# caburu/gym-supplychain

Measured on AMD Instinct MI355X. Metric: env-steps/sec at 65536 envs/GPU, beergame-v0; 1/2/4/8 MI355X, higher is better.
Workload: dtype int32; 1 GPU; beergame-v0 step() x 65536 envs/GPU (BASELINE configs[1]; configs[4] at N=8); n_envs_per_gpu=65536, levels=4, weeks=35, auto_reset=True, ledgers=True, orders_history=True, episode_return_allgather=False, parallelism=env-shard x1

## Files before the change

gym-supplychain_amd/csrc/scg_beergame.hip:

```cpp

#include <cstdarg>
#include <cstdio>
#include <ctime>
#include <vector>

#include "scg_beergame_kernels.h"
#include "scg_server_host.h"

namespace scg {

__global__ __launch_bounds__(kBlock) void poisson_demand_kernel(const BgArgs a, int32_t weeks,
                                                                int32_t* __restrict__ out) {
  const int64_t n = static_cast<int64_t>(blockIdx.x) * kBlock + threadIdx.x;
  if (n >= a.n) return;
  for (int32_t w = 1; w <= weeks; ++w) out[(int64_t)(w - 1) * a.n + n] = week_demand(a, n, w, a.episode);
}

__global__ __launch_bounds__(kBlock) void uniform_ints_kernel(uint32_t k0, uint32_t k1, int64_t env_offset,
                                                              int64_t n_envs, int32_t rows, int32_t width,
                                                              uint32_t tag, int32_t lo, uint32_t range,
                                                              int32_t* __restrict__ out) {
  const int64_t n = static_cast<int64_t>(blockIdx.x) * kBlock + threadIdx.x;
  if (n >= n_envs) return;
  const uint32_t env = static_cast<uint32_t>(env_offset + n);
// ... 19 lines not shown
  if (q < SCG_BG_MAX_LEVELS) dst->init_inv[q] = v.init_inv[q];
  if (q != 63) return;
  dst->env_base = v.env_base;
  dst->pthr_len = v.pthr_len;
  dst->h = v.h;
  dst->b = v.b;
  dst->guard = v.guard;
  dst->demand_lo = v.demand_lo;
  dst->demand_hi = v.demand_hi;
  dst->ship_value = v.ship_value;
  dst->orders_value = v.orders_value;
  dst->init_slots = v.init_slots;
  dst->err_host = v.err_host;
  dst->demand_table = v.demand_table;
  dst->pthr = v.pthr;
}

template <class F>
int with_level(int L, F&& f) {
#define X(l) bg_launchers<l>,
  static const BgLaunchers* (*const kLevels[])() = {SCG_LEVEL_CASES(X)};
#undef X
  if (L < 1 || L > SCG_BG_MAX_LEVELS) return fail(SCG_ERR_INVALID, "levels=%d outside 1..%d", L, SCG_BG_MAX_LEVELS);
  return f(*kLevels[L - 1]());
}

int slab_layout(int L, int64_t N, int32_t R, int32_t T, bool history, int64_t* off) {
  const int64_t NL = N * L;
  if (NL % 4 != 0) return fail(SCG_ERR_INVALID, "slab layout needs n_envs * levels %% 4 == 0 (got %lld)", (long long)NL);
  if (R < 1 || R > static_cast<int32_t>(kSlabRingMax)) return fail(SCG_ERR_INVALID, "slab layout needs 1 <= ring_slots <= 127");
// ... 116 lines not shown
  std::memcpy(w, &v, sizeof(w));
  uint64_t h = 0x9E3779B97F4A7C15ull ^ reinterpret_cast<uintptr_t>(block);
  for (uint64_t x : w) {
    h = (h ^ x) * 0xFF51AFD7ED558CCDull;
    h ^= h >> 29;
  }
  return h | 1u;
}

int sync_slab_consts(const scg_bg_config* cfg, scg_bg_state* st, hipStream_t s) {
  const BgSlabConst v = slab_consts(cfg, st);
  const uint64_t tag = slab_consts_tag(v, st->step_consts);
  if (tag == st->step_consts_tag) return SCG_OK;
  if (reinterpret_cast<uintptr_t>(st->step_consts) % alignof(BgSlabConst) != 0)
    return fail(SCG_ERR_INVALID, "step_consts must be %d-byte aligned", static_cast<int>(alignof(BgSlabConst)));
  hipLaunchKernelGGL(bg_slab_consts_kernel, dim3(1), dim3(64), 0, s, static_cast<BgSlabConst*>(st->step_consts), v);
  if (int rc = check_launch("bg_slab_consts_kernel")) return rc;
  st->step_consts_tag = tag;
  return SCG_OK;
}

}

using namespace scg;

extern "C" {

int scg_bg_struct_sizes(size_t* config_size, size_t* state_size) {
  if (config_size) *config_size = sizeof(scg_bg_config);
  if (state_size) *state_size = sizeof(scg_bg_state);
  return SCG_OK;
// ... 117 lines not shown
  } else {
    st->week = wk.week;
  }
}

static int check_step(const scg_bg_config* cfg, const scg_bg_state* st) {
  if (st->week < 0) return fail(SCG_ERR_NOT_RESET, "step() before reset()");
  if (st->week >= cfg->max_weeks)
    return fail(SCG_ERR_PAST_HORIZON, "step() after the terminal week %d (customer_demand has %d weeks)",
                cfg->max_weeks, cfg->max_weeks);
  return SCG_OK;
}

int scg_bg_step(const scg_bg_config* cfg, scg_bg_state* st, const int32_t* action, int32_t* obs,
                int32_t* reward, int32_t* terminal_obs, uint32_t flags, int32_t* done, void* stream) {
  return scg_bg_step_timed(cfg, st, action, obs, reward, terminal_obs, flags, done, nullptr, nullptr, stream);
}

int scg_bg_step_timed(const scg_bg_config* cfg, scg_bg_state* st, const int32_t* action, int32_t* obs,
                      int32_t* reward, int32_t* terminal_obs, uint32_t flags, int32_t* done, void* start_event,
                      void* stop_event, void* stream) {
  if (int rc = check_state(cfg, st)) return rc;
  if (!action || !obs || !reward) return fail(SCG_ERR_INVALID, "action/obs/reward buffers are required");
  if (int rc = check_step(cfg, st)) return rc;
  const int32_t w = st->week + 1;
  const WeekInfo wk = week_info(cfg, w, flags);
  const dim3 grid = grid_for(st->n_envs);
  const hipStream_t s = static_cast<hipStream_t>(stream);
  const hipEvent_t ev0 = static_cast<hipEvent_t>(start_event), ev1 = static_cast<hipEvent_t>(stop_event);
  if (slab_ready(cfg, st, obs, reward, terminal_obs)) {
    if (int rc = sync_slab_consts(cfg, st, s)) return rc;
    const uint32_t wpack = pack_week_slab(wk, cfg->ring_slots, st->inventory_costs != nullptr,
                                          st->episode_return != nullptr, st->orders_history != nullptr);
    const SlabLaunch sl{st->slab, action, obs, static_cast<const BgSlabConst*>(st->step_consts), st->seed,
                        static_cast<uint32_t>(st->n_envs), wpack, static_cast<uint32_t>(w), st->episode,
                        wk.demand_fixed};
    if (int rc = with_level(cfg->levels, [&](const BgLaunchers& k) { return k.slab(cfg->demand_mode, grid, s, sl, ev0, ev1); }))
      return rc;
  } else {
    BgArgs a = make_args(cfg, st);
    a.act = action;
    a.obs = obs;
    a.rew = reward;
    a.term_obs = terminal_obs;
    if (int rc = with_level(cfg->levels, [&](const BgLaunchers& k) {
          return cfg->variant == 2 ? k.step2(grid, s, a, wk) : k.step(grid, s, a, wk, ev0, ev1);
        }))
      return rc;
  }
  advance_week(st, wk);
  if (done) *done = (wk.flags & WEEK_TERMINAL) ? 1 : 0;
  return SCG_OK;
}

// ... 368 lines not shown
```

gym-supplychain_amd/csrc/scg_beergame_kernels.h:

```cpp
#pragma once

#include <hip/hip_ext.h>
#include <hip/hip_runtime.h>

#include <algorithm>
#include <cmath>
#include <cstdint>
#include <cstdlib>
#include <cstring>
#include <type_traits>

#include "scg_bg_local.h"
#include "scg_bg_mlp.h"
#include "scg_bg_plan.h"
#include "scg_bg_policy.h"
#include "scg_common.h"
#include "scg_mailbox.h"
#include "scg_const.h"
#include "scg_philox.h"
#include "scgpu.h"

namespace scg {

constexpr int kBlock = 256;
// ... 510 lines not shown
  __builtin_amdgcn_fence(__ATOMIC_RELEASE, "");
  if (lane == 0) __hip_atomic_store(&box->exit_seq, ex, __ATOMIC_RELEASE, __HIP_MEMORY_SCOPE_SYSTEM);
}

struct alignas(64) BgSlabConst {
  uint32_t env_base;
  int32_t pthr_len;
  int32_t h, b, guard;
  int32_t demand_lo, demand_hi;
  int32_t ship_value, orders_value, init_slots;
  int32_t* err_host;
  const int32_t* demand_table;
  const uint32_t* pthr;
  int32_t init_inv[SCG_BG_MAX_LEVELS];
  uint32_t thr[kFastThr];
};
static_assert(sizeof(BgSlabConst) <= SCG_BG_STEP_CONSTS_BYTES && offsetof(BgSlabConst, err_host) == 40 &&
                  offsetof(BgSlabConst, init_inv) == 64 && offsetof(BgSlabConst, thr) == 128,
              "BgSlabConst layout");

constexpr int kSlabHeader = 4;

template <int L, int DM>
__global__ __launch_bounds__(kBlock) void bg_step_slab_kernel(int32_t* __restrict__ slab, const int32_t* __restrict__ act_p,
                                                              int32_t* __restrict__ out,
                                                              const BgSlabConst* __restrict__ consts, uint64_t key,
                                                              uint32_t n32, uint32_t wpack, uint32_t week,
                                                              uint32_t episode, int32_t demand_fixed) {
  const int64_t n = static_cast<int64_t>(blockIdx.x) * kBlock + threadIdx.x;
  if (n >= static_cast<int64_t>(n32)) return;
  const ConstTab<BgSlabConst> c = const_tab(consts);
  const uint32_t key0 = static_cast<uint32_t>(key), key1 = static_cast<uint32_t>(key >> 32);
  const WeekPlan p = unpack_week_slab(wpack);
  const int32_t read_slot = p.read_slot, write_slot = p.write_slot, mode = p.mode, R = p.R;
  const bool terminal = p.terminal, autoreset = p.autoreset;
  const bool ledgers = p.ledgers, returns = p.returns, history = p.history;
  const int64_t NL = static_cast<int64_t>(n32) * L;
  const int64_t row = n * L;
  int32_t* const rows = slab + kSlabHeader;
  int32_t* const inv_p = rows, *const bk_p = rows + NL, *const op_p = rows + 2 * NL;
  int32_t* const iacc_p = rows + 3 * NL, *const bacc_p = rows + 4 * NL, *const term_p = rows + 5 * NL;
  int32_t* const ring_p = rows + 6 * NL;
  int64_t* const ret_p = reinterpret_cast<int64_t*>(rows + (6 + R) * NL);
  int64_t* const fret_p = ret_p + n32;
  int32_t* const hist_p = reinterpret_cast<int32_t*>(fret_p + n32);

  int32_t inv[L], bk[L], op[L], act[L], due[L], cur[L], iacc[L], bacc[L];
  zero_row<L>(due);
  zero_row<L>(cur);
  zero_row<L>(iacc);
  zero_row<L>(bacc);
  load_row<L>(inv_p + row, inv);
  load_row<L>(bk_p + row, bk);
  load_row<L>(op_p + row, op);
  load_row<L>(act_p + row, act);
  if (read_slot >= 0) load_row<L>(ring_p + read_slot * NL + row, due);
  if (mode == MODE_ADD) load_row<L>(ring_p + write_slot * NL + row, cur);
  if (ledgers && !autoreset) {
    load_row<L>(iacc_p + row, iacc);
    load_row<L>(bacc_p + row, bacc);
  }
// ... 11 lines not shown
  } else if constexpr (DM == SCG_DEMAND_UNIFORM) {
    const int32_t lo = c->demand_lo, hi = c->demand_hi;
    uint32_t env_base = c->env_base;
    asm volatile("" : "+s"(env_base) : "s"(lo), "s"(hi), "s"(h), "s"(b), "s"(guard), "s"(err_host));
    const uint32_t w = scg::philox_word(key0, key1, env_base + static_cast<uint32_t>(n), episode, week - 1,
                                        SCG_STREAM_BG2_DEMAND);
    demand = lo + static_cast<int32_t>((static_cast<uint64_t>(w) * static_cast<uint32_t>(hi - lo)) >> 32);
  } else {
    static_assert(kFastThr == 40, "the thresholds are read as 16 + 16 + 8 dwords");
    const u32x16 t0 = *reinterpret_cast<ConstTab<u32x16>>(c->thr);
    const u32x16 t1 = *reinterpret_cast<ConstTab<u32x16>>(c->thr + 16);
    const u32x8 t2 = *reinterpret_cast<ConstTab<u32x8>>(c->thr + 32);
    const int32_t len = c->pthr_len;
    const ConstTab<uint32_t> pthr = const_tab(c->pthr);
    uint32_t env_base = c->env_base;
    asm volatile("" : "+s"(env_base) : "s"(t0), "s"(t1), "s"(t2), "s"(len), "s"(pthr), "s"(h), "s"(b), "s"(guard),
                 "s"(err_host));
    uint32_t fast[kFastThr];
#pragma unroll
    for (int q = 0; q < 16; ++q) fast[q] = t0[q], fast[16 + q] = t1[q];
#pragma unroll
    for (int q = 0; q < 8; ++q) fast[32 + q] = t2[q];
    const uint32_t u = scg::philox_word(key0, key1, env_base + static_cast<uint32_t>(n), episode, week - 1,
                                        SCG_STREAM_DEMAND);
    demand = poisson_count_padded(fast, pthr, len, u);
  }
  export_error(n, terminal, slab, err_host);

  int32_t ship[L], obs[L];
  bool ovf = false;
  const int32_t reward = week_update<L>(h, b, guard, demand, mode == MODE_DIRECT, due, inv, bk, op, act, ship,
                                        obs, cur, iacc, bacc, ovf);
  if (mode == MODE_STORE) {
    store_row_p<L>(ring_p + write_slot * NL + row, ship);
  } else if (mode == MODE_ADD) {
    store_row_p<L>(ring_p + write_slot * NL + row, cur);
  }
  out[NL + n] = reward;
  if (history) store_row_p<L>(hist_p + static_cast<int64_t>(week) * NL + row, op);
  const int64_t ret = ret0 + reward;
// ... 646 lines not shown
```

gym-supplychain_amd/csrc/scg_bg_plan.h:

```cpp
#pragma once

#include <cstdint>

#include "scgpu.h"

#if defined(__HIPCC__)
#define SCG_PLAN_HD __host__ __device__ __attribute__((always_inline)) inline
#else
#define SCG_PLAN_HD inline
#endif

namespace scg {

enum : int32_t { MODE_DIRECT = 0, MODE_STORE = 1, MODE_ADD = 2, MODE_DROP = 3 };
constexpr int32_t PLAN_ARRIVE = 4;
inline int32_t plan_mode(int32_t p) { return p & 3; }
inline bool plan_arrive(int32_t p) { return (p & PLAN_ARRIVE) != 0; }
constexpr int kPlanDelayShift = 8;
static_assert(static_cast<int64_t>(SCG_BG_MAX_DELAY) << kPlanDelayShift <= INT32_MAX, "plan delay field too narrow");
inline int32_t plan_word(int32_t mode, bool arrive, int32_t delay) {
  return mode | (arrive ? PLAN_ARRIVE : 0) | (delay << kPlanDelayShift);
}
inline int32_t plan_delay(int32_t p) { return p >> kPlanDelayShift; }

// ... 2 lines not shown
  int32_t week;
  int32_t read_slot;
  int32_t write_slot;
  int32_t mode;
  int32_t demand_fixed;
  int32_t flags;
};

struct WeekPlan {
  int32_t read_slot;
  int32_t write_slot;
  int32_t mode;
  uint32_t terminal, autoreset;
  int32_t R;
  uint32_t ledgers, returns, history;
};

constexpr uint32_t kWeekSlotBits = 14, kWeekSlotMask = (1u << kWeekSlotBits) - 1;
constexpr uint32_t kWeekModeShift = 2 * kWeekSlotBits, kWeekFlagsShift = kWeekModeShift + 2;
static_assert(SCG_BG_MAX_WEEKS + SCG_BG_MAX_DELAY + 2 < (1 << kWeekSlotBits), "ring slot field too narrow");
static_assert(kWeekFlagsShift + 2 == 32 && MODE_DROP <= 3 && (WEEK_TERMINAL | WEEK_AUTORESET) <= 3, "week word fields");
SCG_PLAN_HD uint32_t pack_week(const WeekInfo& wk) {
  return static_cast<uint32_t>(wk.read_slot + 1) | (static_cast<uint32_t>(wk.write_slot) << kWeekSlotBits) |
         (static_cast<uint32_t>(wk.mode) << kWeekModeShift) | (static_cast<uint32_t>(wk.flags) << kWeekFlagsShift);
}
SCG_PLAN_HD WeekPlan unpack_week(uint32_t w) {
  WeekPlan p{};
  p.read_slot = static_cast<int32_t>(w & kWeekSlotMask) - 1;
  p.write_slot = static_cast<int32_t>((w >> kWeekSlotBits) & kWeekSlotMask);
  p.mode = static_cast<int32_t>((w >> kWeekModeShift) & 3u);
  p.terminal = w & (static_cast<uint32_t>(WEEK_TERMINAL) << kWeekFlagsShift);
  p.autoreset = w & (static_cast<uint32_t>(WEEK_AUTORESET) << kWeekFlagsShift);
  return p;
}

constexpr uint32_t kSlabSlotBits = 8, kSlabSlotMask = (1u << kSlabSlotBits) - 1;
constexpr uint32_t kSlabModeShift = 2 * kSlabSlotBits, kSlabRingShift = 24, kSlabRingMax = 127;
constexpr uint32_t SW_TERMINAL = 1u << 18, SW_AUTORESET = 1u << 19, SW_LEDGERS = 1u << 20, SW_RETURNS = 1u << 21,
                   SW_HISTORY = 1u << 22;
static_assert(kSlabRingMax <= kSlabSlotMask && (3u << kSlabModeShift) < SW_TERMINAL &&
                  SW_HISTORY < (1u << kSlabRingShift) && (kSlabRingMax << kSlabRingShift) >> kSlabRingShift == kSlabRingMax,
              "slab week word fields");
SCG_PLAN_HD uint32_t pack_week_slab(const WeekInfo& wk, int32_t R, bool ledgers, bool returns, bool history) {
  return static_cast<uint32_t>(wk.read_slot + 1) | (static_cast<uint32_t>(wk.write_slot) << kSlabSlotBits) |
         (static_cast<uint32_t>(wk.mode) << kSlabModeShift) | ((wk.flags & WEEK_TERMINAL) ? SW_TERMINAL : 0u) |
         ((wk.flags & WEEK_AUTORESET) ? SW_AUTORESET : 0u) | (ledgers ? SW_LEDGERS : 0u) |
         (returns ? SW_RETURNS : 0u) | (history ? SW_HISTORY : 0u) | (static_cast<uint32_t>(R) << kSlabRingShift);
}
SCG_PLAN_HD WeekPlan unpack_week_slab(uint32_t w) {
  WeekPlan p{};
  p.read_slot = static_cast<int32_t>(w & kSlabSlotMask) - 1;
  p.write_slot = static_cast<int32_t>((w >> kSlabSlotBits) & kSlabSlotMask);
  p.mode = static_cast<int32_t>((w >> kSlabModeShift) & 3u);
  p.R = static_cast<int32_t>((w >> kSlabRingShift) & kSlabRingMax);
  p.terminal = w & SW_TERMINAL;
  p.autoreset = w & SW_AUTORESET;
  p.ledgers = w & SW_LEDGERS;
  p.returns = w & SW_RETURNS;
  p.history = w & SW_HISTORY;
  return p;
}

}
```

gym-supplychain_amd/csrc/scg_pybind.c:

```c
#define PY_SSIZE_T_CLEAN
#include <Python.h>
#include <stdint.h>
#include <time.h>

#include "scgpu.h"

static int as_ptr(PyObject* o, void** out) {
  if (o == Py_None) {
    *out = NULL;
    return 0;
  }
  unsigned long long v = PyLong_AsUnsignedLongLong(o);
  if (v == (unsigned long long)-1 && PyErr_Occurred()) return -1;
  *out = (void*)(uintptr_t)v;
  return 0;
}

static PyObject* bg_step(PyObject* self, PyObject* const* args, Py_ssize_t nargs) {
  (void)self;
  void* p[8];
  if (nargs != 8) {
    PyErr_SetString(PyExc_TypeError, "bg_step expects 8 arguments");
    return NULL;
  }
  for (int i = 0; i < 8; ++i)
    if (as_ptr(args[i], &p[i])) return NULL;
  int32_t done = 0;
  const int rc = scg_bg_step((const scg_bg_config*)p[0], (scg_bg_state*)p[1], (const int32_t*)p[2], (int32_t*)p[3],
                             (int32_t*)p[4], (int32_t*)p[5], (uint32_t)(uintptr_t)p[6], &done, p[7]);
  return PyLong_FromLong((long)((rc << 1) | (done ? 1 : 0)));
}

typedef struct bg_step_args {
  uint64_t cfg, state, obs, reward, terminal_obs;
  uint32_t flags;
} bg_step_args;

static PyObject* bg_step_h(PyObject* self, PyObject* const* args, Py_ssize_t nargs) {
  (void)self;
  void* p[3];
  if (nargs != 3) {
    PyErr_SetString(PyExc_TypeError, "bg_step_h expects 3 arguments");
    return NULL;
  }
  for (int i = 0; i < 3; ++i)
    if (as_ptr(args[i], &p[i])) return NULL;
  const bg_step_args* h = (const bg_step_args*)p[0];
  if (!h) {
    PyErr_SetString(PyExc_ValueError, "bg_step_h: null handle");
    return NULL;
  }
  int32_t done = 0;
  const int rc = scg_bg_step((const scg_bg_config*)(uintptr_t)h->cfg, (scg_bg_state*)(uintptr_t)h->state,
                             (const int32_t*)p[1], (int32_t*)(uintptr_t)h->obs, (int32_t*)(uintptr_t)h->reward,
                             (int32_t*)(uintptr_t)h->terminal_obs, h->flags, &done, p[2]);
  return PyLong_FromLong((long)((rc << 1) | (done ? 1 : 0)));
}

static PyObject* bg_step_timed(PyObject* self, PyObject* const* args, Py_ssize_t nargs) {
  (void)self;
  void* p[10];
  if (nargs != 10) {
    PyErr_SetString(PyExc_TypeError, "bg_step_timed expects 10 arguments");
    return NULL;
  }
  for (int i = 0; i < 10; ++i)
    if (as_ptr(args[i], &p[i])) return NULL;
  int32_t done = 0;
  const int rc = scg_bg_step_timed((const scg_bg_config*)p[0], (scg_bg_state*)p[1], (const int32_t*)p[2],
                                   (int32_t*)p[3], (int32_t*)p[4], (int32_t*)p[5], (uint32_t)(uintptr_t)p[6], &done,
                                   p[7], p[8], p[9]);
  return PyLong_FromLong((long)((rc << 1) | (done ? 1 : 0)));
}

static PyObject* bg_server_step(PyObject* self, PyObject* const* args, Py_ssize_t nargs) {
  (void)self;
  void* p[3];
  if (nargs != 3) {
    PyErr_SetString(PyExc_TypeError, "bg_server_step expects 3 arguments");
    return NULL;
  }
  for (int i = 0; i < 3; ++i)
    if (as_ptr(args[i], &p[i])) return NULL;
  scg_bg_state* st = (scg_bg_state*)p[1];
  scg_bg_server_slot* slot = (scg_bg_server_slot*)p[2];
  int32_t done = 0;
// ... 85 lines not shown
      __builtin_ia32_pause();
    }
  }
  Py_END_ALLOW_THREADS
  if (timed_out) {
    PyErr_SetString(PyExc_TimeoutError, "node_barrier: not every rank arrived");
    return NULL;
  }
  return PyLong_FromLong(sense);
}

static PyMethodDef methods[] = {
    {"bg_step", (PyCFunction)(void (*)(void))bg_step, METH_FASTCALL, "scg_bg_step"},
    {"bg_step_h", (PyCFunction)(void (*)(void))bg_step_h, METH_FASTCALL, "scg_bg_step with the fixed arguments behind a handle"},
    {"bg_server_step", (PyCFunction)(void (*)(void))bg_server_step, METH_FASTCALL, "scg_bg_server_step"},
    {"bg_step_timed", (PyCFunction)(void (*)(void))bg_step_timed, METH_FASTCALL, "scg_bg_step_timed"},
    {"sc_step", (PyCFunction)(void (*)(void))sc_step, METH_FASTCALL, "scg_sc_step"},
    {"sc_server_step", (PyCFunction)(void (*)(void))sc_server_step, METH_FASTCALL, "scg_sc_server_post + _wait"},
    {"node_barrier", (PyCFunction)(void (*)(void))node_barrier, METH_FASTCALL, "host barrier of one node's ranks"},
    {NULL, NULL, 0, NULL},
};

static struct PyModuleDef module = {PyModuleDef_HEAD_INIT, "_scgpu_fast", NULL, -1, methods,
                                    NULL, NULL, NULL, NULL};

PyMODINIT_FUNC PyInit__scgpu_fast(void) { return PyModule_Create(&module); }
```

gym-supplychain_amd/gym_supplychain_amd/_native.py:

```python
import ctypes
import os

import torch

LIB_NAME = "libscgpu.so"
LIB_PATH = os.path.join(os.path.dirname(os.path.abspath(__file__)), LIB_NAME)
ABI_VERSION = 9

SCG_OK = 0
SCG_ERR_INVALID = 1
SCG_ERR_PAST_HORIZON = 2
SCG_ERR_NOT_RESET = 3
SCG_ERR_HIP = 4
SCG_PENDING = 5

SCG_DEMAND_FIXED = 0
SCG_DEMAND_TABLE = 1
SCG_DEMAND_POISSON = 2
SCG_DEMAND_UNIFORM = 3

SCG_BG_AUTORESET = 1
SCG_SC_SERIAL = 2
SCG_SC_LAST_OBS = 8
SCG_STREAM_DEMAND = 0
# ... 61 lines not shown
        ("inventory_costs", ctypes.c_void_p),
        ("backlog_costs", ctypes.c_void_p),
        ("orders_history", ctypes.c_void_p),
        ("episode_return", ctypes.c_void_p),
        ("final_return", ctypes.c_void_p),
        ("penalty_costs", ctypes.c_void_p),
        ("error_flags", ctypes.c_void_p),
        ("error_host", ctypes.c_void_p),
        ("slab", ctypes.c_void_p),
        ("step_consts", ctypes.c_void_p),
        ("step_consts_tag", ctypes.c_uint64),
    ]


BG_STEP_CONSTS_BYTES = 512


BG_SERVER_SLOTS = 15
BG_SERVER_ARGS_BYTES = 512


class BgPolicy(ctypes.Structure):
    _fields_ = [("kind", ctypes.c_int32), ("shift", ctypes.c_int32), ("act_lo", ctypes.c_int32),
                ("act_hi", ctypes.c_int32), ("params", ctypes.c_void_p)]


class BgLocalPolicy(ctypes.Structure):
    _fields_ = [("kind", ctypes.c_int32), ("shift", ctypes.c_int32), ("act_lo", ctypes.c_int32),
                ("act_hi", ctypes.c_int32), ("params", ctypes.c_void_p)]

# ... 142 lines not shown
SIGNATURES = {
    "scg_abi_version": (ctypes.c_int, []),
    "scg_last_error": (ctypes.c_char_p, []),
    "scg_bg_struct_sizes": (ctypes.c_int, [ctypes.POINTER(ctypes.c_size_t), ctypes.POINTER(ctypes.c_size_t)]),
    "scg_poisson_table": (ctypes.c_int, [ctypes.c_double, _u32p, ctypes.c_int32]),
    "scg_bg_prepare": (ctypes.c_int, [ctypes.POINTER(BgConfig)]),
    "scg_bg_slab_layout": (ctypes.c_int, [ctypes.POINTER(BgConfig), ctypes.c_int64, ctypes.c_int32, _i64p]),
    "scg_bg_reset": (ctypes.c_int, [ctypes.POINTER(BgConfig), ctypes.POINTER(BgState), ctypes.c_void_p,
                                    ctypes.c_void_p]),
    "scg_bg_step": (ctypes.c_int, [ctypes.POINTER(BgConfig), ctypes.POINTER(BgState), ctypes.c_void_p,
                                   ctypes.c_void_p, ctypes.c_void_p, ctypes.c_void_p, ctypes.c_uint32,
                                   _i32p, ctypes.c_void_p]),
    "scg_bg_step_timed": (ctypes.c_int, [ctypes.POINTER(BgConfig), ctypes.POINTER(BgState), ctypes.c_void_p,
                                         ctypes.c_void_p, ctypes.c_void_p, ctypes.c_void_p, ctypes.c_uint32,
                                         _i32p, ctypes.c_void_p, ctypes.c_void_p, ctypes.c_void_p]),
    "scg_bg_server_attach": (ctypes.c_int, [ctypes.POINTER(BgServer), ctypes.POINTER(BgServerSlot)]),
    "scg_bg_server_detach": (ctypes.c_int, [ctypes.POINTER(BgServerSlot)]),
    "scg_bg_server_post": (ctypes.c_int, [ctypes.POINTER(BgConfig), ctypes.POINTER(BgState),
                                          ctypes.POINTER(BgServerSlot)]),
    "scg_bg_server_wait": (ctypes.c_int, [ctypes.POINTER(BgState), ctypes.POINTER(BgServerSlot), ctypes.c_int64,
                                          _i32p]),
    "scg_bg_server_step": (ctypes.c_int, [ctypes.POINTER(BgConfig), ctypes.POINTER(BgState),
                                          ctypes.POINTER(BgServerSlot), _i32p]),
    "scg_bg_server_stop": (ctypes.c_int, [ctypes.POINTER(BgServer)]),
    "scg_bg_server_line_check": (ctypes.c_uint32, [ctypes.POINTER(BgServerLine)]),
    "scg_bg_rollout": (ctypes.c_int, [ctypes.POINTER(BgConfig), ctypes.POINTER(BgState), ctypes.c_int32,
                                      ctypes.c_void_p, ctypes.c_void_p, ctypes.c_void_p, ctypes.c_uint32,
                                      ctypes.c_void_p]),
    "scg_bg_rollout_policy": (ctypes.c_int, [ctypes.POINTER(BgConfig), ctypes.POINTER(BgState), ctypes.c_int32,
                                             ctypes.POINTER(BgPolicy), ctypes.c_void_p, ctypes.c_void_p,
# ... 109 lines not shown
    buf = (ctypes.c_uint32 * POISSON_MAX)()
    n = lib.scg_poisson_table(float(lam), buf, POISSON_MAX)
    if n < 0:
        check(-n)
    return list(buf[:n])


try:
    _raw_stream = torch._C._cuda_getCurrentRawStream
except AttributeError:
    _raw_stream = None


class BgStepArgs(ctypes.Structure):
    _fields_ = [("cfg", ctypes.c_uint64), ("state", ctypes.c_uint64), ("obs", ctypes.c_uint64),
                ("reward", ctypes.c_uint64), ("terminal_obs", ctypes.c_uint64), ("flags", ctypes.c_uint32)]


def raw_stream(device_index):
    if _raw_stream is not None:
        return _raw_stream(device_index)
    return torch.cuda.current_stream(device_index).cuda_stream


def raw_stream_fn():
    return _raw_stream if _raw_stream is not None else raw_stream


_hip = None


# ... 111 lines not shown
```

gym-supplychain_amd/gym_supplychain_amd/envs/beergame_env.py:

```python
import ctypes
import numbers
import os
import threading
import weakref

import numpy as np
import torch

from .. import _native as nat
from .. import checkpoint as ckpt
from .. import spaces
from . import resident
from .step_server import _ResidentServer
from .supplychain_env import SupplyChainVecEnv, pack_mlp_words
from ..distributed import entropy_seed

STD_LEVELS = 4
STD_DEMAND = [4] * 4 + [8] * 31
STD_INVENTORY = 12
STD_SHIP_DELAY = 2
STD_SHIP_VALUE = 4
STD_ORDERS_VALUE = 4
STD_INV_COST = 1
STD_BACKLOG_COST = 2
# ... 196 lines not shown
            self._final_ret = i64(nat.SLAB_FINAL_RETURN) if track_returns else None
            self._term_obs = rows(nat.SLAB_TERMINAL_OBS)
        else:
            self._err = torch.zeros(1, **i32)
            self._inv = torch.zeros((n_envs, L), **i32)
            self._bk = torch.zeros((n_envs, L), **i32)
            self._op = torch.zeros((n_envs, L), **i32)
            self._ring = torch.zeros((R, n_envs, L), **i32)
            self._inv_costs = torch.zeros((n_envs, L), **i32) if track_costs else None
            self._bk_costs = torch.zeros((n_envs, L), **i32) if track_costs else None
            self._hist = torch.zeros((T + 1, n_envs, L), **i32) if track_history else None
            self._ret = torch.zeros(n_envs, dtype=torch.int64, device=dev) if track_returns else None
            self._final_ret = torch.zeros(n_envs, dtype=torch.int64, device=dev) if track_returns else None
            self._term_obs = torch.zeros((n_envs, L), **i32)
        self._pen_costs = torch.zeros((n_envs, L), **i32) if (track_costs and v2) else None
        self._out = torch.zeros(n_envs * L + n_envs, **i32)
        self._obs = self._out[: n_envs * L].view(n_envs, L)
        self._rew = self._out[n_envs * L:]
        self._done_false = torch.zeros(n_envs, dtype=torch.bool, device=dev)
        self._done_true = torch.ones(n_envs, dtype=torch.bool, device=dev)
        self._err_word = nat.MappedWord()

        s = nat.BgState()
        s.n_envs, s.env_offset, s.seed = n_envs, int(env_offset), int(seed) & 0xFFFFFFFFFFFFFFFF
        s.episode, s.week = 0, -1
        s.inventory, s.backlog, s.orders_placed = self._inv.data_ptr(), self._bk.data_ptr(), self._op.data_ptr()
        s.shipments = self._ring.data_ptr()
        s.inventory_costs = self._inv_costs.data_ptr() if track_costs else None
        s.backlog_costs = self._bk_costs.data_ptr() if track_costs else None
        s.orders_history = self._hist.data_ptr() if track_history else None
        s.episode_return = self._ret.data_ptr() if track_returns else None
# ... 1 lines not shown
        s.penalty_costs = self._pen_costs.data_ptr() if self._pen_costs is not None else None
        s.error_flags = self._err.data_ptr()
        s.error_host = self._err_word.dev
        s.slab = self._slab.data_ptr() if self._slab is not None else None
        s.step_consts = self._step_consts.data_ptr() if self._step_consts is not None else None
        s.step_consts_tag = 0
        self._st = s
        self._cfg_ref = ctypes.byref(self._cfg)
        self._st_ref = ctypes.byref(self._st)
        self._done_flag = ctypes.c_int32(0)
        self._done_ref = ctypes.byref(self._done_flag)
        self._flags = nat.SCG_BG_AUTORESET if self.auto_reset else 0
        self._act_shape = (n_envs, L)
        self._obs_ptr, self._rew_ptr = self._obs.data_ptr(), self._rew.data_ptr()
        self._term_ptr = self._term_obs.data_ptr()
        self._cfg_addr, self._st_addr = ctypes.addressof(self._cfg), ctypes.addressof(self._st)
        self._fast_step, self._fast_step_timed = nat.fast.bg_step, nat.fast.bg_step_timed
        self._step_args = nat.BgStepArgs(self._cfg_addr, self._st_addr, self._obs_ptr, self._rew_ptr, self._term_ptr,
                                         self._flags)
        self._step_handle = ctypes.addressof(self._step_args)
        self._fast_step_h = nat.fast.bg_step_h
        self._raw_stream = nat.raw_stream_fn()
        self._ready = {}
        self._act_numel = n_envs * L
        self.single_observation_space = spaces.Box(_I32[0], _I32[1], (L,), np.int32)
        self.single_action_space = spaces.Box(-ACTION_BOUND, ACTION_BOUND - 1, (L,), np.int32)
        self.observation_space = spaces.Box(_I32[0], _I32[1], (n_envs, L), np.int32)
        self.action_space = spaces.Box(-ACTION_BOUND, ACTION_BOUND - 1, (n_envs, L), np.int32)

    def _stream(self):
        return nat.raw_stream(self._dev_index)

    def reset(self):
        nat.check(nat.lib.scg_bg_reset(self._cfg_ref, self._st_ref, self._obs.data_ptr(), self._stream()))
# ... 27 lines not shown
                and actions.numel() == self._act_numel:
            ptr = ok[1]
        else:
            if self._is_ready(actions):
                if len(self._ready) >= 64:
                    self._ready.clear()
                self._ready[id(actions)] = (weakref.ref(actions), actions.data_ptr())
            else:
                actions = self._actions(actions)
            ptr = actions.data_ptr()
        if _events is None:
            r = self._fast_step_h(self._step_handle, ptr, self._raw_stream(self._dev_index))
        else:
            r = self._fast_step_timed(self._cfg_addr, self._st_addr, ptr, self._obs_ptr,
                                      self._rew_ptr, self._term_ptr, self._flags, _events[0], _events[1],
                                      nat.raw_stream(self._dev_index))
        if r > 1:
            nat.check(r >> 1)
        if r & 1:
            self._poll_errors()
            info = {"terminal_observation": self._term_obs}
            if self._final_ret is not None:
                info["episode_return"] = self._final_ret
            return self._obs, self._rew, self._done_true, info
        return self._obs, self._rew, self._done_false, {}

    def _poll_errors(self):
        if self._err_word.value:
            raise OverflowError("a BeerGame value left int32 range (the reference's int64 state would differ); "
                                "results since then are invalid")

# ... 352 lines not shown
        self.initial_orders_value = cfg.initial_orders_value
        self.current_state = None
        ra = (4 * L + 15) // 16 * 16
        self._io = io = nat.MappedBuffer(16 + ra + 4 * (L + 1))
        self._err_np = io.view(np.int32, 0, 1)
        self._act_np = io.view(np.int32, 16, L)
        self._out_np = io.view(np.int32, 16 + ra, L + 1)
        self._act_dev = io.dev + 16
        vec = self._vec
        vec._st.error_flags = io.dev
        vec._err = torch.from_numpy(self._err_np)
        obs_dev, rew_dev = io.dev + 16 + ra, io.dev + 16 + ra + 4 * L
        self._server = None
        if os.environ.get("SCG_BG_SERVER", "1") != "0":
            self._server = _StepServer.attach(self._vec, self._act_dev, io.host + 16, obs_dev, rew_dev)
        self._step_args = nat.BgStepArgs(vec._cfg_addr, vec._st_addr, obs_dev, rew_dev, vec._term_ptr, 0)
        self._handle = ctypes.addressof(self._step_args)
        self._fast_step_h = nat.fast.bg_step_h
        self._sync = nat.stream_synchronize_fn()
        self._last_act = None
        self.week = None

    def reset(self):
        obs = self._vec.reset()
        self.week = 0
        self._last_act = None
        self.current_state = obs[0].cpu().numpy().astype(np.int64)
        return self.current_state

    def step(self, action):
        if self.week is None:
# ... 271 lines not shown
```

include/scgpu.h:

```cpp
#ifndef SCGPU_H
#define SCGPU_H

#include <stddef.h>
#include <stdint.h>

#ifdef __cplusplus
extern "C" {
#endif

#define SCG_ABI_VERSION 9

#if defined(__GNUC__)
#define SCG_API __attribute__((visibility("default")))
#else
#define SCG_API
#endif

#define SCG_BG_MAX_LEVELS 16
#define SCG_BG_MAX_WEEKS 4096
#define SCG_BG_MAX_DELAY 4096
#define SCG_POISSON_MAX 256
#define SCG_BG_ROLLOUT_MAX 128

typedef enum scg_status {
// ... 98 lines not shown

SCG_API int scg_bg_prepare(scg_bg_config* cfg);

SCG_API int scg_bg_slab_layout(const scg_bg_config* cfg, int64_t n_envs, int32_t with_history,
                               int64_t offsets[SCG_SLAB_FIELDS]);

SCG_API int scg_bg_reset(const scg_bg_config* cfg, scg_bg_state* st, int32_t* obs, void* stream);

SCG_API int scg_bg_step(const scg_bg_config* cfg, scg_bg_state* st, const int32_t* action,
                int32_t* obs, int32_t* reward, int32_t* terminal_obs, uint32_t flags,
                int32_t* done, void* stream);

SCG_API int scg_bg_step_timed(const scg_bg_config* cfg, scg_bg_state* st, const int32_t* action,
                              int32_t* obs, int32_t* reward, int32_t* terminal_obs, uint32_t flags,
                              int32_t* done, void* start_event, void* stop_event, void* stream);

#define SCG_BG_SERVER_SLOTS 15
#define SCG_BG_SERVER_ARGS_BYTES 512
#define SCG_PENDING 5

typedef struct scg_bg_server_line {
  uint32_t req_seq;
  int32_t cmd;
  uint32_t wpack;
  int32_t week;
  int32_t demand_fixed;
  int32_t n_inline;
  uint32_t gen;
  uint32_t check;
  int32_t action[8];
// ... 326 lines not shown
```

Baseline: 15.34 billion env-steps/s.

## Precompute next week's Poisson demand in extra blocks of the step kernel

The slab step kernel is launched with twice the grid for Poisson demand. The extra blocks draw the next week's demand into a double-banked 'ahead' buffer, tagged with key, env base, episode, week and an upload stamp. On the next step the main blocks check the tag and reuse the pre-drawn value, falling back to the inline Philox+Poisson draw on a mismatch. This takes the RNG and inverse-CDF work off the step's critical path, at the cost of more blocks per launch, an extra global read per env, and added tag-validation complexity.

```diff
diff --git a/gym-supplychain_amd/csrc/scg_beergame.hip b/gym-supplychain_amd/csrc/scg_beergame.hip
--- a/gym-supplychain_amd/csrc/scg_beergame.hip
+++ b/gym-supplychain_amd/csrc/scg_beergame.hip
@@ -1,4 +1,5 @@
 
+#include <atomic>
 #include <cstdarg>
 #include <cstdio>
 #include <ctime>
@@ -57,6 +58,7 @@
   dst->err_host = v.err_host;
   dst->demand_table = v.demand_table;
   dst->pthr = v.pthr;
+  dst->stamp = v.stamp;
 }
 
 template <class F>
@@ -203,7 +205,10 @@
   if (tag == st->step_consts_tag) return SCG_OK;
   if (reinterpret_cast<uintptr_t>(st->step_consts) % alignof(BgSlabConst) != 0)
     return fail(SCG_ERR_INVALID, "step_consts must be %d-byte aligned", static_cast<int>(alignof(BgSlabConst)));
-  hipLaunchKernelGGL(bg_slab_consts_kernel, dim3(1), dim3(64), 0, s, static_cast<BgSlabConst*>(st->step_consts), v);
+  static std::atomic<uint32_t> uploads{0};
+  BgSlabConst up = v;
+  do up.stamp = uploads.fetch_add(1, std::memory_order_relaxed) + 1; while (up.stamp == 0);
+  hipLaunchKernelGGL(bg_slab_consts_kernel, dim3(1), dim3(64), 0, s, static_cast<BgSlabConst*>(st->step_consts), up);
   if (int rc = check_launch("bg_slab_consts_kernel")) return rc;
   st->step_consts_tag = tag;
   return SCG_OK;
@@ -351,30 +356,42 @@
 
 int scg_bg_step(const scg_bg_config* cfg, scg_bg_state* st, const int32_t* action, int32_t* obs,
                 int32_t* reward, int32_t* terminal_obs, uint32_t flags, int32_t* done, void* stream) {
-  return scg_bg_step_timed(cfg, st, action, obs, reward, terminal_obs, flags, done, nullptr, nullptr, stream);
+  return scg_bg_step_ex(cfg, st, action, obs, reward, terminal_obs, flags, done, nullptr, nullptr, nullptr, stream);
 }
 
 int scg_bg_step_timed(const scg_bg_config* cfg, scg_bg_state* st, const int32_t* action, int32_t* obs,
                       int32_t* reward, int32_t* terminal_obs, uint32_t flags, int32_t* done, void* start_event,
                       void* stop_event, void* stream) {
+  return scg_bg_step_ex(cfg, st, action, obs, reward, terminal_obs, flags, done, start_event, stop_event, nullptr,
+                        stream);
+}
+
+int scg_bg_step_ex(const scg_bg_config* cfg, scg_bg_state* st, const int32_t* action, int32_t* obs,
+                   int32_t* reward, int32_t* terminal_obs, uint32_t flags, int32_t* done, void* start_event,
+                   void* stop_event, int32_t* ahead, void* stream) {
   if (int rc = check_state(cfg, st)) return rc;
   if (!action || !obs || !reward) return fail(SCG_ERR_INVALID, "action/obs/reward buffers are required");
   if (int rc = check_step(cfg, st)) return rc;
   const int32_t w = st->week + 1;
   const WeekInfo wk = week_info(cfg, w, flags);
-  const dim3 grid = grid_for(st->n_envs);
   const hipStream_t s = static_cast<hipStream_t>(stream);
   const hipEvent_t ev0 = static_cast<hipEvent_t>(start_event), ev1 = static_cast<hipEvent_t>(stop_event);
   if (slab_ready(cfg, st, obs, reward, terminal_obs)) {
     if (int rc = sync_slab_consts(cfg, st, s)) return rc;
+    const bool rows = ahead && ahead == reward + st->n_envs && cfg->demand_mode == SCG_DEMAND_POISSON &&
+                      st->n_envs <= kAheadMaxEnvs;
     const uint32_t wpack = pack_week_slab(wk, cfg->ring_slots, st->inventory_costs != nullptr,
-                                          st->episode_return != nullptr, st->orders_history != nullptr);
+                                          st->episode_return != nullptr, st->orders_history != nullptr, rows,
+                                          demand_bank(st->episode, cfg->max_weeks, w));
+    const bool draw = rows && !((wk.flags & WEEK_TERMINAL) && !(wk.flags & WEEK_AUTORESET));
+    const dim3 grid(draw ? 2 * grid_for(st->n_envs).x : grid_for(st->n_envs).x);
     const SlabLaunch sl{st->slab, action, obs, static_cast<const BgSlabConst*>(st->step_consts), st->seed,
                         static_cast<uint32_t>(st->n_envs), wpack, static_cast<uint32_t>(w), st->episode,
                         wk.demand_fixed};
     if (int rc = with_level(cfg->levels, [&](const BgLaunchers& k) { return k.slab(cfg->demand_mode, grid, s, sl, ev0, ev1); }))
       return rc;
   } else {
+    const dim3 grid = grid_for(st->n_envs);
     BgArgs a = make_args(cfg, st);
     a.act = action;
     a.obs = obs;
diff --git a/gym-supplychain_amd/csrc/scg_beergame_kernels.h b/gym-supplychain_amd/csrc/scg_beergame_kernels.h
--- a/gym-supplychain_amd/csrc/scg_beergame_kernels.h
+++ b/gym-supplychain_amd/csrc/scg_beergame_kernels.h
@@ -548,12 +548,52 @@
   const uint32_t* pthr;
   int32_t init_inv[SCG_BG_MAX_LEVELS];
   uint32_t thr[kFastThr];
+  uint32_t stamp;
 };
 static_assert(sizeof(BgSlabConst) <= SCG_BG_STEP_CONSTS_BYTES && offsetof(BgSlabConst, err_host) == 40 &&
-                  offsetof(BgSlabConst, init_inv) == 64 && offsetof(BgSlabConst, thr) == 128,
+                  offsetof(BgSlabConst, init_inv) == 64 && offsetof(BgSlabConst, thr) == 128 &&
+                  offsetof(BgSlabConst, stamp) == 288 && sizeof(BgSlabConst) == 320,
               "BgSlabConst layout");
 
 constexpr int kSlabHeader = 4;
+
+constexpr int kAheadHeader = SCG_BG_AHEAD_HEADER, kAheadTagWords = 7, kAheadPathWord = SCG_BG_AHEAD_PATH_WORD;
+enum : int { TAG_KEY0 = 0, TAG_KEY1, TAG_ENV_BASE, TAG_N, TAG_EPISODE, TAG_WEEK, TAG_STAMP };
+constexpr int64_t kAheadMaxEnvs = 65536;
+static_assert(8 + kAheadTagWords <= kAheadPathWord && kAheadPathWord < kAheadHeader, "two tags and the path word");
+
+__device__ __forceinline__ void draw_ahead(ConstTab<BgSlabConst> c, int32_t* __restrict__ ahead, uint32_t key0,
+                                           uint32_t key1, uint32_t n32, const WeekPlan& p, uint32_t week,
+                                           uint32_t episode, int64_t n) {
+  if (n >= static_cast<int64_t>(n32)) return;
+  static_assert(kFastThr == 40, "the thresholds are read as 16 + 16 + 8 dwords");
+  const u32x16 t0 = *reinterpret_cast<ConstTab<u32x16>>(c->thr);
+  const u32x16 t1 = *reinterpret_cast<ConstTab<u32x16>>(c->thr + 16);
+  const u32x8 t2 = *reinterpret_cast<ConstTab<u32x8>>(c->thr + 32);
+  const int32_t len = c->pthr_len;
+  const ConstTab<uint32_t> pthr = const_tab(c->pthr);
+  const uint32_t env_base = c->env_base, stamp = c->stamp;
+  const uint32_t next_week = p.terminal ? 1u : week + 1, next_episode = p.terminal ? episode + 1 : episode;
+  uint32_t fast[kFastThr];
+#pragma unroll
+  for (int q = 0; q < 16; ++q) fast[q] = t0[q], fast[16 + q] = t1[q];
+#pragma unroll
+  for (int q = 0; q < 8; ++q) fast[32 + q] = t2[q];
+  const uint32_t u = scg::philox_word(key0, key1, env_base + static_cast<uint32_t>(n), next_episode, next_week - 1,
+                                      SCG_STREAM_DEMAND);
+  const uint32_t bank = p.bank ^ 1u;
+  ahead[kAheadHeader + static_cast<int64_t>(bank) * n32 + n] = poisson_count_padded(fast, pthr, len, u);
+  if (n == 0) {
+    uint32_t* const tag = reinterpret_cast<uint32_t*>(ahead) + 8 * bank;
+    tag[TAG_KEY0] = key0;
+    tag[TAG_KEY1] = key1;
+    tag[TAG_ENV_BASE] = env_base;
+    tag[TAG_N] = n32;
+    tag[TAG_EPISODE] = next_episode;
+    tag[TAG_WEEK] = next_week;
+    tag[TAG_STAMP] = stamp;
+  }
+}
 
 template <int L, int DM>
 __global__ __launch_bounds__(kBlock) void bg_step_slab_kernel(int32_t* __restrict__ slab, const int32_t* __restrict__ act_p,
@@ -561,11 +601,19 @@
                                                               const BgSlabConst* __restrict__ consts, uint64_t key,
                                                               uint32_t n32, uint32_t wpack, uint32_t week,
                                                               uint32_t episode, int32_t demand_fixed) {
-  const int64_t n = static_cast<int64_t>(blockIdx.x) * kBlock + threadIdx.x;
-  if (n >= static_cast<int64_t>(n32)) return;
   const ConstTab<BgSlabConst> c = const_tab(consts);
   const uint32_t key0 = static_cast<uint32_t>(key), key1 = static_cast<uint32_t>(key >> 32);
   const WeekPlan p = unpack_week_slab(wpack);
+  int32_t* const ahead = out + (static_cast<int64_t>(n32) * L + n32);
+  if constexpr (DM == SCG_DEMAND_POISSON) {
+    const uint32_t G = (n32 + kBlock - 1) / kBlock;
+    if (blockIdx.x >= G) {
+      draw_ahead(c, ahead, key0, key1, n32, p, week, episode, static_cast<int64_t>(blockIdx.x - G) * kBlock + threadIdx.x);
+      return;
+    }
+  }
+  const int64_t n = static_cast<int64_t>(blockIdx.x) * kBlock + threadIdx.x;
+  if (n >= static_cast<int64_t>(n32)) return;
   const int32_t read_slot = p.read_slot, write_slot = p.write_slot, mode = p.mode, R = p.R;
   const bool terminal = p.terminal, autoreset = p.autoreset;
   const bool ledgers = p.ledgers, returns = p.returns, history = p.history;
@@ -579,6 +627,9 @@
   int64_t* const fret_p = ret_p + n32;
   int32_t* const hist_p = reinterpret_cast<int32_t*>(fret_p + n32);
 
+  int32_t drawn = 0;
+  if constexpr (DM == SCG_DEMAND_POISSON)
+    if (p.ahead) drawn = ahead[kAheadHeader + static_cast<int64_t>(p.bank) * n32 + n];
   int32_t inv[L], bk[L], op[L], act[L], due[L], cur[L], iacc[L], bacc[L];
   zero_row<L>(due);
   zero_row<L>(cur);
@@ -620,16 +671,27 @@
     const int32_t len = c->pthr_len;
     const ConstTab<uint32_t> pthr = const_tab(c->pthr);
     uint32_t env_base = c->env_base;
+    const uint32_t stamp = c->stamp;
+    const u32x8 tag = *reinterpret_cast<ConstTab<u32x8>>(
+        p.ahead ? const_tab(reinterpret_cast<const uint32_t*>(ahead) + 8 * p.bank) : static_cast<ConstTab<uint32_t>>(c->thr));
     asm volatile("" : "+s"(env_base) : "s"(t0), "s"(t1), "s"(t2), "s"(len), "s"(pthr), "s"(h), "s"(b), "s"(guard),
-                 "s"(err_host));
-    uint32_t fast[kFastThr];
-#pragma unroll
-    for (int q = 0; q < 16; ++q) fast[q] = t0[q], fast[16 + q] = t1[q];
-#pragma unroll
-    for (int q = 0; q < 8; ++q) fast[32 + q] = t2[q];
-    const uint32_t u = scg::philox_word(key0, key1, env_base + static_cast<uint32_t>(n), episode, week - 1,
-                                        SCG_STREAM_DEMAND);
-    demand = poisson_count_padded(fast, pthr, len, u);
+                 "s"(err_host), "s"(stamp), "s"(tag));
+    const uint32_t miss = (tag[TAG_KEY0] ^ key0) | (tag[TAG_KEY1] ^ key1) | (tag[TAG_ENV_BASE] ^ env_base) |
+                          (tag[TAG_N] ^ n32) | (tag[TAG_EPISODE] ^ episode) | (tag[TAG_WEEK] ^ week) |
+                          (tag[TAG_STAMP] ^ stamp) | (p.ahead ^ SW_AHEAD);
+    if (miss == 0) {
+      demand = drawn;
+    } else {
+      uint32_t fast[kFastThr];
+#pragma unroll
+      for (int q = 0; q < 16; ++q) fast[q] = t0[q], fast[16 + q] = t1[q];
+#pragma unroll
+      for (int q = 0; q < 8; ++q) fast[32 + q] = t2[q];
+      const uint32_t u = scg::philox_word(key0, key1, env_base + static_cast<uint32_t>(n), episode, week - 1,
+                                          SCG_STREAM_DEMAND);
+      demand = poisson_count_padded(fast, pthr, len, u);
+    }
+    if (p.ahead && n == 0) ahead[kAheadPathWord] = miss == 0 ? 1 : 0;
   }
   export_error(n, terminal, slab, err_host);
 
diff --git a/gym-supplychain_amd/csrc/scg_bg_plan.h b/gym-supplychain_amd/csrc/scg_bg_plan.h
--- a/gym-supplychain_amd/csrc/scg_bg_plan.h
+++ b/gym-supplychain_amd/csrc/scg_bg_plan.h
@@ -40,6 +40,7 @@
   uint32_t terminal, autoreset;
   int32_t R;
   uint32_t ledgers, returns, history;
+  uint32_t ahead, bank;
 };
 
 constexpr uint32_t kWeekSlotBits = 14, kWeekSlotMask = (1u << kWeekSlotBits) - 1;
@@ -63,15 +64,23 @@
 constexpr uint32_t kSlabSlotBits = 8, kSlabSlotMask = (1u << kSlabSlotBits) - 1;
 constexpr uint32_t kSlabModeShift = 2 * kSlabSlotBits, kSlabRingShift = 24, kSlabRingMax = 127;
 constexpr uint32_t SW_TERMINAL = 1u << 18, SW_AUTORESET = 1u << 19, SW_LEDGERS = 1u << 20, SW_RETURNS = 1u << 21,
-                   SW_HISTORY = 1u << 22;
+                   SW_HISTORY = 1u << 22, SW_AHEAD = 1u << 23, SW_BANK = 1u << 31;
 static_assert(kSlabRingMax <= kSlabSlotMask && (3u << kSlabModeShift) < SW_TERMINAL &&
                   SW_HISTORY < (1u << kSlabRingShift) && (kSlabRingMax << kSlabRingShift) >> kSlabRingShift == kSlabRingMax,
               "slab week word fields");
-SCG_PLAN_HD uint32_t pack_week_slab(const WeekInfo& wk, int32_t R, bool ledgers, bool returns, bool history) {
+static_assert(SW_HISTORY < SW_AHEAD && SW_AHEAD < (1u << kSlabRingShift) &&
+                  ((kSlabRingMax << kSlabRingShift) & SW_BANK) == 0 && SW_BANK == 1u << 31,
+              "slab week word: the demand-row bits lie between the SW_* bits and R, and above R");
+SCG_PLAN_HD uint32_t demand_bank(uint32_t episode, int32_t max_weeks, int32_t week) {
+  return (episode * static_cast<uint32_t>(max_weeks) + static_cast<uint32_t>(week)) & 1u;
+}
+SCG_PLAN_HD uint32_t pack_week_slab(const WeekInfo& wk, int32_t R, bool ledgers, bool returns, bool history,
+                                    bool ahead = false, uint32_t bank = 0) {
   return static_cast<uint32_t>(wk.read_slot + 1) | (static_cast<uint32_t>(wk.write_slot) << kSlabSlotBits) |
          (static_cast<uint32_t>(wk.mode) << kSlabModeShift) | ((wk.flags & WEEK_TERMINAL) ? SW_TERMINAL : 0u) |
          ((wk.flags & WEEK_AUTORESET) ? SW_AUTORESET : 0u) | (ledgers ? SW_LEDGERS : 0u) |
-         (returns ? SW_RETURNS : 0u) | (history ? SW_HISTORY : 0u) | (static_cast<uint32_t>(R) << kSlabRingShift);
+         (returns ? SW_RETURNS : 0u) | (history ? SW_HISTORY : 0u) | (ahead ? SW_AHEAD : 0u) |
+         ((bank & 1u) ? SW_BANK : 0u) | (static_cast<uint32_t>(R) << kSlabRingShift);
 }
 SCG_PLAN_HD WeekPlan unpack_week_slab(uint32_t w) {
   WeekPlan p{};
@@ -84,6 +93,8 @@
   p.ledgers = w & SW_LEDGERS;
   p.returns = w & SW_RETURNS;
   p.history = w & SW_HISTORY;
+  p.ahead = w & SW_AHEAD;
+  p.bank = w >> 31;
   return p;
 }
 
diff --git a/gym-supplychain_amd/csrc/scg_pybind.c b/gym-supplychain_amd/csrc/scg_pybind.c
--- a/gym-supplychain_amd/csrc/scg_pybind.c
+++ b/gym-supplychain_amd/csrc/scg_pybind.c
@@ -34,6 +34,7 @@
 typedef struct bg_step_args {
   uint64_t cfg, state, obs, reward, terminal_obs;
   uint32_t flags;
+  uint64_t ahead;
 } bg_step_args;
 
 static PyObject* bg_step_h(PyObject* self, PyObject* const* args, Py_ssize_t nargs) {
@@ -51,25 +52,26 @@
     return NULL;
   }
   int32_t done = 0;
-  const int rc = scg_bg_step((const scg_bg_config*)(uintptr_t)h->cfg, (scg_bg_state*)(uintptr_t)h->state,
-                             (const int32_t*)p[1], (int32_t*)(uintptr_t)h->obs, (int32_t*)(uintptr_t)h->reward,
-                             (int32_t*)(uintptr_t)h->terminal_obs, h->flags, &done, p[2]);
+  const int rc = scg_bg_step_ex((const scg_bg_config*)(uintptr_t)h->cfg, (scg_bg_state*)(uintptr_t)h->state,
+                                (const int32_t*)p[1], (int32_t*)(uintptr_t)h->obs, (int32_t*)(uintptr_t)h->reward,
+                                (int32_t*)(uintptr_t)h->terminal_obs, h->flags, &done, NULL, NULL,
+                                (int32_t*)(uintptr_t)h->ahead, p[2]);
   return PyLong_FromLong((long)((rc << 1) | (done ? 1 : 0)));
 }
 
 static PyObject* bg_step_timed(PyObject* self, PyObject* const* args, Py_ssize_t nargs) {
   (void)self;
-  void* p[10];
-  if (nargs != 10) {
-    PyErr_SetString(PyExc_TypeError, "bg_step_timed expects 10 arguments");
-    return NULL;
-  }
-  for (int i = 0; i < 10; ++i)
-    if (as_ptr(args[i], &p[i])) return NULL;
-  int32_t done = 0;
-  const int rc = scg_bg_step_timed((const scg_bg_config*)p[0], (scg_bg_state*)p[1], (const int32_t*)p[2],
-                                   (int32_t*)p[3], (int32_t*)p[4], (int32_t*)p[5], (uint32_t)(uintptr_t)p[6], &done,
-                                   p[7], p[8], p[9]);
+  void* p[11];
+  if (nargs != 11) {
+    PyErr_SetString(PyExc_TypeError, "bg_step_timed expects 11 arguments");
+    return NULL;
+  }
+  for (int i = 0; i < 11; ++i)
+    if (as_ptr(args[i], &p[i])) return NULL;
+  int32_t done = 0;
+  const int rc = scg_bg_step_ex((const scg_bg_config*)p[0], (scg_bg_state*)p[1], (const int32_t*)p[2],
+                                (int32_t*)p[3], (int32_t*)p[4], (int32_t*)p[5], (uint32_t)(uintptr_t)p[6], &done,
+                                p[7], p[8], (int32_t*)p[9], p[10]);
   return PyLong_FromLong((long)((rc << 1) | (done ? 1 : 0)));
 }
 
@@ -185,7 +187,7 @@
     {"bg_step", (PyCFunction)(void (*)(void))bg_step, METH_FASTCALL, "scg_bg_step"},
     {"bg_step_h", (PyCFunction)(void (*)(void))bg_step_h, METH_FASTCALL, "scg_bg_step with the fixed arguments behind a handle"},
     {"bg_server_step", (PyCFunction)(void (*)(void))bg_server_step, METH_FASTCALL, "scg_bg_server_step"},
-    {"bg_step_timed", (PyCFunction)(void (*)(void))bg_step_timed, METH_FASTCALL, "scg_bg_step_timed"},
+    {"bg_step_timed", (PyCFunction)(void (*)(void))bg_step_timed, METH_FASTCALL, "scg_bg_step_ex"},
     {"sc_step", (PyCFunction)(void (*)(void))sc_step, METH_FASTCALL, "scg_sc_step"},
     {"sc_server_step", (PyCFunction)(void (*)(void))sc_server_step, METH_FASTCALL, "scg_sc_server_post + _wait"},
     {"node_barrier", (PyCFunction)(void (*)(void))node_barrier, METH_FASTCALL, "host barrier of one node's ranks"},
diff --git a/gym-supplychain_amd/gym_supplychain_amd/_native.py b/gym-supplychain_amd/gym_supplychain_amd/_native.py
--- a/gym-supplychain_amd/gym_supplychain_amd/_native.py
+++ b/gym-supplychain_amd/gym_supplychain_amd/_native.py
@@ -99,6 +99,8 @@
 
 
 BG_STEP_CONSTS_BYTES = 512
+BG_AHEAD_HEADER = 16
+BG_AHEAD_PATH_WORD = 15
 
 
 BG_SERVER_SLOTS = 15
@@ -271,6 +273,9 @@
     "scg_bg_step_timed": (ctypes.c_int, [ctypes.POINTER(BgConfig), ctypes.POINTER(BgState), ctypes.c_void_p,
                                          ctypes.c_void_p, ctypes.c_void_p, ctypes.c_void_p, ctypes.c_uint32,
                                          _i32p, ctypes.c_void_p, ctypes.c_void_p, ctypes.c_void_p]),
+    "scg_bg_step_ex": (ctypes.c_int, [ctypes.POINTER(BgConfig), ctypes.POINTER(BgState), ctypes.c_void_p,
+                                      ctypes.c_void_p, ctypes.c_void_p, ctypes.c_void_p, ctypes.c_uint32,
+                                      _i32p, ctypes.c_void_p, ctypes.c_void_p, ctypes.c_void_p, ctypes.c_void_p]),
     "scg_bg_server_attach": (ctypes.c_int, [ctypes.POINTER(BgServer), ctypes.POINTER(BgServerSlot)]),
     "scg_bg_server_detach": (ctypes.c_int, [ctypes.POINTER(BgServerSlot)]),
     "scg_bg_server_post": (ctypes.c_int, [ctypes.POINTER(BgConfig), ctypes.POINTER(BgState),
@@ -410,7 +415,8 @@
 
 class BgStepArgs(ctypes.Structure):
     _fields_ = [("cfg", ctypes.c_uint64), ("state", ctypes.c_uint64), ("obs", ctypes.c_uint64),
-                ("reward", ctypes.c_uint64), ("terminal_obs", ctypes.c_uint64), ("flags", ctypes.c_uint32)]
+                ("reward", ctypes.c_uint64), ("terminal_obs", ctypes.c_uint64), ("flags", ctypes.c_uint32),
+                ("ahead", ctypes.c_uint64)]
 
 
 def raw_stream(device_index):
diff --git a/gym-supplychain_amd/gym_supplychain_amd/envs/beergame_env.py b/gym-supplychain_amd/gym_supplychain_amd/envs/beergame_env.py
--- a/gym-supplychain_amd/gym_supplychain_amd/envs/beergame_env.py
+++ b/gym-supplychain_amd/gym_supplychain_amd/envs/beergame_env.py
@@ -234,7 +234,13 @@
             self._final_ret = torch.zeros(n_envs, dtype=torch.int64, device=dev) if track_returns else None
             self._term_obs = torch.zeros((n_envs, L), **i32)
         self._pen_costs = torch.zeros((n_envs, L), **i32) if (track_costs and v2) else None
-        self._out = torch.zeros(n_envs * L + n_envs, **i32)
+        self._ahead = None
+        if self._slab is not None and mode == nat.SCG_DEMAND_POISSON and not v2:
+            backing = torch.zeros(n_envs * L + n_envs + nat.BG_AHEAD_HEADER + 2 * n_envs, **i32)
+            self._out = backing[: n_envs * L + n_envs]
+            self._ahead = backing[n_envs * L + n_envs:]
+        else:
+            self._out = torch.zeros(n_envs * L + n_envs, **i32)
         self._obs = self._out[: n_envs * L].view(n_envs, L)
         self._rew = self._out[n_envs * L:]
         self._done_false = torch.zeros(n_envs, dtype=torch.bool, device=dev)
@@ -266,10 +272,11 @@
         self._act_shape = (n_envs, L)
         self._obs_ptr, self._rew_ptr = self._obs.data_ptr(), self._rew.data_ptr()
         self._term_ptr = self._term_obs.data_ptr()
+        self._ahead_ptr = self._ahead.data_ptr() if self._ahead is not None else None
         self._cfg_addr, self._st_addr = ctypes.addressof(self._cfg), ctypes.addressof(self._st)
         self._fast_step, self._fast_step_timed = nat.fast.bg_step, nat.fast.bg_step_timed
         self._step_args = nat.BgStepArgs(self._cfg_addr, self._st_addr, self._obs_ptr, self._rew_ptr, self._term_ptr,
-                                         self._flags)
+                                         self._flags, self._ahead_ptr or 0)
         self._step_handle = ctypes.addressof(self._step_args)
         self._fast_step_h = nat.fast.bg_step_h
         self._raw_stream = nat.raw_stream_fn()
@@ -327,7 +334,7 @@
         else:
             r = self._fast_step_timed(self._cfg_addr, self._st_addr, ptr, self._obs_ptr,
                                       self._rew_ptr, self._term_ptr, self._flags, _events[0], _events[1],
-                                      nat.raw_stream(self._dev_index))
+                                      self._ahead_ptr, nat.raw_stream(self._dev_index))
         if r > 1:
             nat.check(r >> 1)
         if r & 1:
@@ -710,7 +717,7 @@
         self._server = None
         if os.environ.get("SCG_BG_SERVER", "1") != "0":
             self._server = _StepServer.attach(self._vec, self._act_dev, io.host + 16, obs_dev, rew_dev)
-        self._step_args = nat.BgStepArgs(vec._cfg_addr, vec._st_addr, obs_dev, rew_dev, vec._term_ptr, 0)
+        self._step_args = nat.BgStepArgs(vec._cfg_addr, vec._st_addr, obs_dev, rew_dev, vec._term_ptr, 0, 0)
         self._handle = ctypes.addressof(self._step_args)
         self._fast_step_h = nat.fast.bg_step_h
         self._sync = nat.stream_synchronize_fn()
diff --git a/include/scgpu.h b/include/scgpu.h
--- a/include/scgpu.h
+++ b/include/scgpu.h
@@ -136,6 +136,13 @@
 SCG_API int scg_bg_step_timed(const scg_bg_config* cfg, scg_bg_state* st, const int32_t* action,
                               int32_t* obs, int32_t* reward, int32_t* terminal_obs, uint32_t flags,
                               int32_t* done, void* start_event, void* stop_event, void* stream);
+
+#define SCG_BG_AHEAD_HEADER 16
+#define SCG_BG_AHEAD_PATH_WORD 15
+SCG_API int scg_bg_step_ex(const scg_bg_config* cfg, scg_bg_state* st, const int32_t* action,
+                           int32_t* obs, int32_t* reward, int32_t* terminal_obs, uint32_t flags,
+                           int32_t* done, void* start_event, void* stop_event, int32_t* ahead,
+                           void* stream);
 
 #define SCG_BG_SERVER_SLOTS 15
 #define SCG_BG_SERVER_ARGS_BYTES 512
```

Measured after the change: 16.05 billion env-steps/s, median of 6. 4.6% higher.
